# pyscf/pyscf

Measured on AMD Instinct MI355X. Metric: ms per SCF iter (DF J/K build), lower is better.
Workload: dtype f64

## Files before the change

pyscf_amd/csrc/xc_sparse.hip:

```cpp
#include <algorithm>
#include <type_traits>
#include <vector>
#include "common.h"
#include "mfma_e2.h"

using namespace pamd;

static int g_orb_dot_dma = 1;
static int g_orb_rho_128 = 1;
static int g_orb_rho_fused = 1;
static int g_vmat_probe = 0;
static int g_vmat_burst = 0;
static int g_vmat_even = 1;
static int g_vmat_flip = 0;
static int g_vmat_xcd = 1;

namespace {

struct SubTiles {
    const long *ao_off;
    const long *aow_off;
    const long *idx_off;
    const int *ld;
    const int *idx;
};


__device__ __forceinline__ int xcd_contiguous(int b, int n, int enabled)
{
    if (!enabled || n < 16) return b;
    const int q = n >> 3, r = n & 7, x = b & 7, slot = b >> 3;
    return x < r ? x * (q + 1) + slot : r * (q + 1) + (x - r) * q + slot;
}

template <int MT>
__global__ __launch_bounds__(256, 2) void sub_orb_dot_kernel(const double *__restrict__ ao_c, SubTiles tl, int G, int nchunk,
                                                             const double *__restrict__ orb, int ldo, int nocc_pad,
                                                             double *__restrict__ cmo, long comp_stride, long ldc)
{
    const int t = blockIdx.z / nchunk, chunk = blockIdx.z - t * nchunk;
    const int ld = tl.ld[t];
    const double *src = ao_c + tl.ao_off[t] + (long)blockIdx.y * G * ld;
    double *out = cmo + (long)blockIdx.y * comp_stride + (long)t * G;
    e2_symm_body<MT, true, true>(src, ld, ld, orb, ldo, out, nocc_pad, ldc, G, nullptr, nullptr, tl.idx + tl.idx_off[t],
                                 blockIdx.x * NT, chunk * (MT * 16));
}

__global__ __launch_bounds__(256, 2) void sub_orb_dot2_kernel(const double *__restrict__ ao_c, SubTiles tl, int G, int nchunk,
                                                              const double *__restrict__ orb, int ldo, int nocc_pad,
                                                              double *__restrict__ cmo, long comp_stride, long ldc)
{
    __shared__ double sa0[KB * LDN + KB * 32];
    __shared__ double sa1[KB * LDN + KB * 32];
    __shared__ double sq0[KB * LDN];
    __shared__ double sq1[KB * LDN];
    constexpr int RB = KB * LDN;
    const int tid = threadIdx.x, lane = tid & 63;
    const int wave = __builtin_amdgcn_readfirstlane(tid >> 6);
    const int t = blockIdx.z / nchunk, chunk = blockIdx.z - t * nchunk;
    const int ld = tl.ld[t];
    const int n0 = blockIdx.x * NT, m0 = chunk * 160;
    const int *idx = tl.idx + tl.idx_off[t];
    const __amdgpu_buffer_rsrc_t r_b = __builtin_amdgcn_make_buffer_rsrc(
        (void *)(ao_c + tl.ao_off[t] + ((long)blockIdx.y * G + n0) * ld), 0, 0xffffffff, 0x00020000);
    const __amdgpu_buffer_rsrc_t r_orb = __builtin_amdgcn_make_buffer_rsrc((void *)(orb + m0), 0, 0xffffffff, 0x00020000);
    const int ldo8 = ldo * 8;
    const int voff = lane * 16;
    const int rrow = lane >> 4;
    const int voff_remcol = (128 + ((((lane & 15) * 2) - 16 * (rrow & 1)) & 31)) * 8;
    const int wr = wave >> 1, wc = wave & 1;
    const int fk = lane >> 4, fn = lane & 15;
    const int offa = fk * LDN + wr * 64 + fn;
    const int offr = RB + fk * 32 + ((wr * 16 + fn + 16 * (fk & 1)) & 31);
    const int pl = fn & 7, bodd = (fn >> 3) & 1;
    const int offb_tr = (wc * 8 + (fn >> 3)) * 128 + (((pl ^ bodd) * 8) + ((fk >> 1) ^ (pl & 1))) * 2 + (fk & 1);
    int atr[4];
#pragma unroll
    for (int g = 0; g < 4; g++) atr[g] = offb_tr + (((2 * g) ^ (pl & 6))) * 2;
    int voff_tr[4];
#pragma unroll
    for (int j = 0; j < 4; j++) {
        const int blk = wave * 4 + j;
        const int pl_s = (lane >> 3) ^ (blk & 1);
        const int kp = (lane & 7) ^ pl_s;
        voff_tr[j] = ((blk * 8 + pl_s) * ld + 2 * kp) * 8;
    }

    double4_t acc[5][4];
#pragma unroll
    for (int a = 0; a < 5; a++)
#pragma unroll
        for (int b = 0; b < 4; b++) acc[a][b] = double4_t{0, 0, 0, 0};

    auto stage_row = [&](int k0, double *da, double *db, int j) {
        const int k = wave * 4 + j;
        const int row = idx[k0 + k];
        __builtin_amdgcn_raw_ptr_buffer_load_lds(r_orb, (__attribute__((address_space(3))) void *)(da + k * LDN), 16, voff, row * ldo8, 0, 0);
        __builtin_amdgcn_raw_ptr_buffer_load_lds(r_b, (__attribute__((address_space(3))) void *)(db + k * 128), 16, voff_tr[j], k0 * 8, 0, 0);
        if (j == 0) {
            const int rowl = idx[k0 + wave * 4 + rrow];
            __builtin_amdgcn_raw_ptr_buffer_load_lds(r_orb, (__attribute__((address_space(3))) void *)(da + RB + wave * 128), 16,
                                                     rowl * ldo8 + voff_remcol, 0, 0, 0);
        }
    };
    auto step = [&](const double *ca, const double *cb, double *na, double *nb, int k0) {
        asm volatile("s_waitcnt vmcnt(0)" ::: "memory");
        __syncthreads();
        const int kn = (k0 + KB < ld) ? k0 + KB : k0;
#pragma unroll
        for (int kk = 0; kk < KB; kk += 4) {
            double af[5], bf[4];
#pragma unroll
            for (int a = 0; a < 4; a++) af[a] = ca[offa + kk * LDN + a * 16];
            af[4] = ca[offr + kk * 32];
#pragma unroll
            for (int b = 0; b < 4; b++) bf[b] = cb[atr[kk >> 2] + b * 256];
            stage_row(kn, na, nb, kk >> 2);
#pragma unroll
            for (int a = 0; a < 5; a++)
#pragma unroll
                for (int b = 0; b < 4; b++) acc[a][b] = mfma_f64_16x16x4(af[a], bf[b], acc[a][b]);
        }
    };
#pragma unroll
    for (int j = 0; j < 4; j++) stage_row(0, sa0, sq0, j);
    for (int k0 = 0; k0 < ld; k0 += 2 * KB) {
        step(sa0, sq0, sa1, sq1, k0);
        if (k0 + KB < ld) step(sa1, sq1, sa0, sq0, k0 + KB);
    }
    double *out = cmo + (long)blockIdx.y * comp_stride + (long)t * G;
#pragma unroll
    for (int a = 0; a < 5; a++)
#pragma unroll
        for (int b = 0; b < 4; b++) {
            const int n = n0 + wc * 64 + b * 16 + fn;
            if (n >= G) continue;
#pragma unroll
            for (int r = 0; r < 4; r++) {
                const int i = m0 + (a < 4 ? wr * 64 + a * 16 : 128 + wr * 16) + fk + 4 * r;
                if (i < nocc_pad) out[(long)i * ldc + n] = acc[a][b][r];
            }
        }
}

template <bool REM>
__global__ __launch_bounds__(256, 2) void sub_orb_rho_kernel(const double *__restrict__ ao_c, SubTiles tl, int G, int nchunk,
                                                             const double *__restrict__ orb, int ldo, int nocc,
                                                             const double *__restrict__ sign, double *__restrict__ rho, long ldg)
{
    constexpr int NA = REM ? 5 : 4, CW = REM ? 160 : 128;
    __shared__ double sa0[KB * LDN + KB * 32];
    __shared__ double sa1[KB * LDN + KB * 32];
    __shared__ double sq0[KB * LDN];
    __shared__ double sq1[KB * LDN];
    constexpr int RB = KB * LDN;
    const int tid = threadIdx.x, lane = tid & 63;
    const int wave = __builtin_amdgcn_readfirstlane(tid >> 6);
    const int t = blockIdx.z / nchunk, chunk = blockIdx.z - t * nchunk;
    const int ld = tl.ld[t];
    const int g0 = blockIdx.x * 32, m0 = chunk * CW;
    const int *idx = tl.idx + tl.idx_off[t];
    const __amdgpu_buffer_rsrc_t r_b = __builtin_amdgcn_make_buffer_rsrc((void *)(ao_c + tl.ao_off[t] + (long)g0 * ld), 0, 0xffffffff,
                                                                        0x00020000);
    const __amdgpu_buffer_rsrc_t r_orb = __builtin_amdgcn_make_buffer_rsrc((void *)(orb + m0), 0, 0xffffffff, 0x00020000);
    const int ldo8 = ldo * 8;
    const int voff = lane * 16;
    const int rrow = lane >> 4;
    const int voff_remcol = (128 + ((((lane & 15) * 2) - 16 * (rrow & 1)) & 31)) * 8;
    const int wr = wave >> 1, wc = wave & 1;
    const int fk = lane >> 4, fn = lane & 15;
    const int offa = fk * LDN + wr * 64 + fn;
    const int offr = RB + fk * 32 + ((wr * 16 + fn + 16 * (fk & 1)) & 31);
    const int pl = fn & 7, bodd = (fn >> 3) & 1;
    const int offb_tr = (wc * 8 + (fn >> 3)) * 128 + (((pl ^ bodd) * 8) + ((fk >> 1) ^ (pl & 1))) * 2 + (fk & 1);
    int atr[4];
#pragma unroll
    for (int g = 0; g < 4; g++) atr[g] = offb_tr + (((2 * g) ^ (pl & 6))) * 2;
    int voff_tr[4];
#pragma unroll
    for (int j = 0; j < 4; j++) {
        const int blk = wave * 4 + j;
        const int pl_s = (lane >> 3) ^ (blk & 1);
        const int kp = (lane & 7) ^ pl_s;
        const int n = blk * 8 + pl_s;
        const int comp = (n >> 4) & 3, pt = ((n >> 6) << 4) | (n & 15);
        voff_tr[j] = (int)((((long)comp * G + pt) * ld + 2 * kp) * 8);
    }

    double4_t acc[NA][4];
#pragma unroll
    for (int a = 0; a < NA; a++)
#pragma unroll
        for (int b = 0; b < 4; b++) acc[a][b] = double4_t{0, 0, 0, 0};

    auto stage_row = [&](int k0, double *da, double *db, int j) {
        const int k = wave * 4 + j;
        const int row = idx[k0 + k];
        __builtin_amdgcn_raw_ptr_buffer_load_lds(r_orb, (__attribute__((address_space(3))) void *)(da + k * LDN), 16, voff, row * ldo8, 0, 0);
        __builtin_amdgcn_raw_ptr_buffer_load_lds(r_b, (__attribute__((address_space(3))) void *)(db + k * 128), 16, voff_tr[j], k0 * 8, 0, 0);
        if (REM && j == 0) {
            const int rowl = idx[k0 + wave * 4 + rrow];
            __builtin_amdgcn_raw_ptr_buffer_load_lds(r_orb, (__attribute__((address_space(3))) void *)(da + RB + wave * 128), 16,
                                                     rowl * ldo8 + voff_remcol, 0, 0, 0);
        }
    };
    auto step = [&](const double *ca, const double *cb, double *na, double *nb, int k0) {
        asm volatile("s_waitcnt vmcnt(0)" ::: "memory");
        __syncthreads();
        const int kn = (k0 + KB < ld) ? k0 + KB : k0;
#pragma unroll
        for (int kk = 0; kk < KB; kk += 4) {
            double af[NA], bf[4];
#pragma unroll
            for (int a = 0; a < 4; a++) af[a] = ca[offa + kk * LDN + a * 16];
            if (REM) af[NA - 1] = ca[offr + kk * 32];
#pragma unroll
            for (int b = 0; b < 4; b++) bf[b] = cb[atr[kk >> 2] + b * 256];
            stage_row(kn, na, nb, kk >> 2);
#pragma unroll
            for (int a = 0; a < NA; a++)
#pragma unroll
                for (int b = 0; b < 4; b++) acc[a][b] = mfma_f64_16x16x4(af[a], bf[b], acc[a][b]);
        }
    };
#pragma unroll
    for (int j = 0; j < 4; j++) stage_row(0, sa0, sq0, j);
    for (int k0 = 0; k0 < ld; k0 += 2 * KB) {
        step(sa0, sq0, sa1, sq1, k0);
        if (k0 + KB < ld) step(sa1, sq1, sa0, sq0, k0 + KB);
    }
    double p0 = 0, px = 0, py = 0, pz = 0;
#pragma unroll
    for (int a = 0; a < NA; a++)
#pragma unroll
        for (int r = 0; r < 4; r++) {
            const int i = m0 + (a < 4 ? wr * 64 + a * 16 : 128 + wr * 16) + fk + 4 * r;
            const double c0 = acc[a][0][r];
            const double w = (sign != nullptr && i < nocc) ? sign[i] * c0 : c0;
            p0 += w * c0;
            px += w * acc[a][1][r];
            py += w * acc[a][2][r];
            pz += w * acc[a][3][r];
        }
#pragma unroll
    for (int off = 16; off < 64; off <<= 1) {
        p0 += __shfl_xor(p0, off, 64);
        px += __shfl_xor(px, off, 64);
        py += __shfl_xor(py, off, 64);
        pz += __shfl_xor(pz, off, 64);
    }
    asm volatile("s_waitcnt vmcnt(0)" ::: "memory");
    __syncthreads();
    double *part = sa0;
    if (fk == 0) {
        part[(wave * 4 + 0) * 16 + fn] = p0;
        part[(wave * 4 + 1) * 16 + fn] = 2.0 * px;
        part[(wave * 4 + 2) * 16 + fn] = 2.0 * py;
        part[(wave * 4 + 3) * 16 + fn] = 2.0 * pz;
    }
    __syncthreads();
    if (tid < 128) {
        const int c = tid >> 5, pt = tid & 31, wcol = pt >> 4, f = pt & 15;
        const double v = part[((0 * 2 + wcol) * 4 + c) * 16 + f] + part[((1 * 2 + wcol) * 4 + c) * 16 + f];
        double *dst = rho + (long)c * ldg + (long)t * G + g0 + pt;
        if (nchunk == 1) *dst = v;
        else unsafeAtomicAdd(dst, v);
    }
}

__global__ __launch_bounds__(256) void sub_scale_kernel(const double *__restrict__ ao_c, SubTiles tl, int G, int ncomp,
                                                        const double *__restrict__ wv, long ldg, double *__restrict__ aow_c)
{
    const int t = blockIdx.z;
    const int ld = tl.ld[t];
    const int m = blockIdx.x * 256 + threadIdx.x;
    if (m >= ld) return;
    const long g = blockIdx.y;
    const double *a = ao_c + tl.ao_off[t] + g * ld + m;
    const long cs = (long)G * ld;
    const long gg = (long)t * G + g;
    double v = wv[gg] * a[0];
    if (ncomp == 4) v += wv[ldg + gg] * a[cs] + wv[2 * ldg + gg] * a[2 * cs] + wv[3 * ldg + gg] * a[3 * cs];
    aow_c[tl.aow_off[t] + g * ld + m] = v;
}

__global__ __launch_bounds__(256, 2) void sub_vmat_kernel(const double *__restrict__ ao_c, const double *__restrict__ aow_c,
                                                          SubTiles tl, const int *__restrict__ work, int G, int nao,
                                                          double *__restrict__ vmat, long ldv, int xcd)
{
    __shared__ double sb0[2 * KB * LDN];
    __shared__ double sb1[2 * KB * LDN];
    constexpr int PA = KB * LDN;
    const int tid = threadIdx.x, lane = tid & 63;
    const int wave = __builtin_amdgcn_readfirstlane(tid >> 6);
    const int item = xcd_contiguous(blockIdx.x, gridDim.x, xcd);
    const int t = work[3 * item], tm = work[3 * item + 1], tn = work[3 * item + 2];
    const int ld = tl.ld[t];
    const int p0 = tm * NT, q0 = tn * NT;
    const __amdgpu_buffer_rsrc_t r_a = __builtin_amdgcn_make_buffer_rsrc((void *)(ao_c + tl.ao_off[t] + p0), 0, 0xffffffff, 0x00020000);
    const __amdgpu_buffer_rsrc_t r_b = __builtin_amdgcn_make_buffer_rsrc((void *)(aow_c + tl.aow_off[t] + q0), 0, 0xffffffff, 0x00020000);
    const int voff = lane * 16, ld8 = ld * 8;
    const int wr = wave >> 1, wc = wave & 1;
    const int fk = lane >> 4, fn = lane & 15;
    const int offa = fk * LDN + wr * 64 + fn, offb = PA + fk * LDN + wc * 64 + fn;

    int na = (ld - (p0 + wr * 64) + 15) / 16, nb = (ld - (q0 + wc * 64) + 15) / 16;
    na = na < 0 ? 0 : (na > 4 ? 4 : na);
    nb = nb < 0 ? 0 : (nb > 4 ? 4 : nb);

    double4_t acc[4][4];
#pragma unroll
    for (int a = 0; a < 4; a++)
#pragma unroll
        for (int b = 0; b < 4; b++) acc[a][b] = double4_t{0, 0, 0, 0};

    auto stage_row = [&](int k0, double *dst, int j) {
        const int k = wave * 4 + j;
        __builtin_amdgcn_raw_ptr_buffer_load_lds(r_a, (__attribute__((address_space(3))) void *)(dst + k * LDN), 16, voff, (k0 + k) * ld8, 0, 0);
        __builtin_amdgcn_raw_ptr_buffer_load_lds(r_b, (__attribute__((address_space(3))) void *)(dst + PA + k * LDN), 16, voff, (k0 + k) * ld8, 0, 0);
    };
    auto kloop = [&](auto NAc, auto NBc) {
        constexpr int NA = decltype(NAc)::value, NB = decltype(NBc)::value;
        auto step = [&](const double *cur, double *nxt, int k0) {
            asm volatile("s_waitcnt vmcnt(0)" ::: "memory");
            __syncthreads();
            const int kn = (k0 + KB < G) ? k0 + KB : k0;
#pragma unroll
            for (int kk = 0; kk < KB; kk += 4) {
                double af[4], bf[4];
#pragma unroll
                for (int a = 0; a < NA; a++) af[a] = cur[offa + kk * LDN + a * 16];
#pragma unroll
                for (int b = 0; b < NB; b++) bf[b] = cur[offb + kk * LDN + b * 16];
                stage_row(kn, nxt, kk >> 2);
#pragma unroll
                for (int a = 0; a < NA; a++)
#pragma unroll
                    for (int b = 0; b < NB; b++) acc[a][b] = mfma_f64_16x16x4(af[a], bf[b], acc[a][b]);
            }
        };
        for (int k0 = 0; k0 < G; k0 += 2 * KB) {
            step(sb0, sb1, k0);
            if (k0 + KB < G) step(sb1, sb0, k0 + KB);
        }
    };
#pragma unroll
    for (int j = 0; j < 4; j++) stage_row(0, sb0, j);
    using I0 = std::integral_constant<int, 0>;
    using I1 = std::integral_constant<int, 1>;
    using I2 = std::integral_constant<int, 2>;
    using I3 = std::integral_constant<int, 3>;
    using I4 = std::integral_constant<int, 4>;
    auto pick_b = [&](auto NAc) {
        switch (nb) {
        case 1: kloop(NAc, I1{}); break;
        case 2: kloop(NAc, I2{}); break;
        case 3: kloop(NAc, I3{}); break;
        default: kloop(NAc, I4{}); break;
        }
    };
    if (na == 0 || nb == 0) {
        kloop(I0{}, I0{});
        asm volatile("s_waitcnt vmcnt(0)" ::: "memory");
        return;
    }
    switch (na) {
    case 1: pick_b(I1{}); break;
    case 2: pick_b(I2{}); break;
    case 3: pick_b(I3{}); break;
    default: pick_b(I4{}); break;
    }
    const int *idx = tl.idx + tl.idx_off[t];
#pragma unroll
    for (int b = 0; b < 4; b++) {
        const int col = q0 + wc * 64 + b * 16 + fn;
        if (col >= ld) continue;
        const int aj = idx[col];
        if (aj >= nao) continue;
#pragma unroll
        for (int a = 0; a < 4; a++)
#pragma unroll
            for (int r = 0; r < 4; r++) {
                const int rowi = p0 + wr * 64 + a * 16 + fk + 4 * r;
                if (rowi >= ld) continue;
                const int ai = idx[rowi];
                if (ai < nao) unsafeAtomicAdd(vmat + (long)ai * ldv + aj, acc[a][b][r]);
            }
    }
}

template <bool BURST, int PROBE>
__global__ __launch_bounds__(256, 2) void sub_vmat_sym_kernel(const double *__restrict__ ao_c, const double *__restrict__ aow_c,
                                                              SubTiles tl, const int *__restrict__ work, int G, int nao,
                                                              double *__restrict__ vmat, long ldv, int flip)
{
    __shared__ double sb0[2 * KB * LDN];
    __shared__ double sb1[2 * KB * LDN];
    constexpr int PA = KB * LDN;
    const int tid = threadIdx.x, lane = tid & 63;
    const int wave = __builtin_amdgcn_readfirstlane(tid >> 6);
    const int *w = work + 6 * (long)blockIdx.x;
    const int t = w[0], p0 = w[1], gp = w[2], q0 = w[3], gq = w[4], diag = w[5];
    if (gp == 0) return;
    const int ld = tl.ld[t];
    const int voff = lane * 16, ld8 = ld * 8;
    const int role = wave ^ ((flip == 1 ? (blockIdx.x >> 3) & 1 : flip == 2 ? (blockIdx.x >> 8) & 1 : 0) ? 3 : 0);
    const int wr = role >> 1, wc = role & 1;
    const int fk = lane >> 4, fn = lane & 15;
    const int ga0 = (gp + 1) >> 1, gb0 = (gq + 1) >> 1;
    const int na = wr == 0 ? ga0 : gp - ga0, nb = wc == 0 ? gb0 : gq - gb0;
    const int ra = wr * ga0 * 16, cb = wc * gb0 * 16;
    const int offa = fk * LDN + ra + fn, offb = PA + fk * LDN + cb + fn;
    const double *A = ao_c + tl.ao_off[t], *W = aow_c + tl.aow_off[t];
    const int nphase = diag ? 1 : 2;

    double4_t acc[4][4];
#pragma unroll
    for (int a = 0; a < 4; a++)
#pragma unroll
        for (int b = 0; b < 4; b++) acc[a][b] = double4_t{0, 0, 0, 0};

    auto kloop = [&](auto NAc, auto NBc) {
        constexpr int NA = decltype(NAc)::value, NB = decltype(NBc)::value;
        for (int ph = 0; ph < nphase; ph++) {
            const __amdgpu_buffer_rsrc_t r_a = __builtin_amdgcn_make_buffer_rsrc((void *)((ph ? W : A) + p0), 0, 0xffffffff, 0x00020000);
            const __amdgpu_buffer_rsrc_t r_b = __builtin_amdgcn_make_buffer_rsrc((void *)((ph ? A : W) + q0), 0, 0xffffffff, 0x00020000);
            auto stage_row = [&](int k0, double *dst, int j) {
                const int k = wave * 4 + j;
                __builtin_amdgcn_raw_ptr_buffer_load_lds(r_a, (__attribute__((address_space(3))) void *)(dst + k * LDN), 16, voff, (k0 + k) * ld8, 0, 0);
                __builtin_amdgcn_raw_ptr_buffer_load_lds(r_b, (__attribute__((address_space(3))) void *)(dst + PA + k * LDN), 16, voff, (k0 + k) * ld8, 0, 0);
            };
            auto step = [&](const double *cur, double *nxt, int k0) {
                asm volatile("s_waitcnt vmcnt(0)" ::: "memory");
                __syncthreads();
                const int kn = (k0 + KB < G) ? k0 + KB : k0;
#pragma unroll
                for (int kk = 0; kk < KB; kk += 4) {
                    double af[4], bf[4];
#pragma unroll
                    for (int a = 0; a < NA; a++) af[a] = cur[offa + kk * LDN + a * 16];
#pragma unroll
                    for (int b = 0; b < NB; b++) bf[b] = cur[offb + kk * LDN + b * 16];
                    if (PROBE == 2) {
                    } else if (BURST) {
                        if (kk == 0) {
#pragma unroll
                            for (int j = 0; j < 4; j++) stage_row(kn, nxt, j);
                        }
                    } else {
                        stage_row(kn, nxt, kk >> 2);
                    }
                    if (PROBE == 3) {
                        acc[0][0][0] += af[0] + bf[0];
                        continue;
                    }
#pragma unroll
                    for (int a = 0; a < NA; a++)
#pragma unroll
                        for (int b = 0; b < NB; b++) acc[a][b] = mfma_f64_16x16x4(af[a], bf[b], acc[a][b]);
                }
            };
            __syncthreads();
#pragma unroll
            for (int j = 0; j < 4; j++) stage_row(0, sb0, j);
            for (int k0 = 0; k0 < G; k0 += 2 * KB) {
                step(sb0, sb1, k0);
                if (k0 + KB < G) step(sb1, sb0, k0 + KB);
            }
            asm volatile("s_waitcnt vmcnt(0)" ::: "memory");
        }
    };
    using I0 = std::integral_constant<int, 0>;
    using I1 = std::integral_constant<int, 1>;
    using I2 = std::integral_constant<int, 2>;
    using I3 = std::integral_constant<int, 3>;
    using I4 = std::integral_constant<int, 4>;
    auto pick_b = [&](auto NAc) {
        switch (nb) {
        case 1: kloop(NAc, I1{}); break;
        case 2: kloop(NAc, I2{}); break;
        case 3: kloop(NAc, I3{}); break;
        default: kloop(NAc, I4{}); break;
        }
    };
    if (na <= 0 || nb <= 0) {
        kloop(I0{}, I0{});
        return;
    }
    switch (na) {
    case 1: pick_b(I1{}); break;
    case 2: pick_b(I2{}); break;
    case 3: pick_b(I3{}); break;
    default: pick_b(I4{}); break;
    }
    if (PROBE == 1) {
        double sum = 0;
#pragma unroll
        for (int a = 0; a < 4; a++)
#pragma unroll
            for (int b = 0; b < 4; b++) sum += acc[a][b][0] + acc[a][b][1] + acc[a][b][2] + acc[a][b][3];
        if (sum == 1.2345e300) vmat[0] = 1;
        return;
    }
    const int *idx = tl.idx + tl.idx_off[t];
#pragma unroll
    for (int b = 0; b < 4; b++) {
        if (b >= nb) continue;
        const int col = q0 + cb + b * 16 + fn;
        if (col >= ld) continue;
        const int aj = idx[col];
        if (aj >= nao) continue;
#pragma unroll
        for (int a = 0; a < 4; a++) {
            if (a >= na) continue;
#pragma unroll
            for (int r = 0; r < 4; r++) {
                const int rowi = p0 + ra + a * 16 + fk + 4 * r;
                if (rowi >= ld) continue;
                const int ai = idx[rowi];
                if (ai >= nao) continue;
                if (!diag) unsafeAtomicAdd(vmat + (long)ai * ldv + aj, acc[a][b][r]);
                else if (rowi > col) unsafeAtomicAdd(vmat + (long)ai * ldv + aj, acc[a][b][r]);
                else if (rowi < col) unsafeAtomicAdd(vmat + (long)aj * ldv + ai, acc[a][b][r]);
                else unsafeAtomicAdd(vmat + (long)ai * ldv + aj, 2.0 * acc[a][b][r]);
            }
        }
    }
}

__global__ void mirror_tril_kernel(const double *__restrict__ part, int m, int ldc, double *__restrict__ out)
{
    const int j = blockIdx.x * blockDim.x + threadIdx.x;
    const int i = blockIdx.y;
    if (j >= m) return;
    out[(long)i * m + j] = i >= j ? part[(long)i * ldc + j] : part[(long)j * ldc + i];
}

__global__ __launch_bounds__(256) void sub_gather_kernel(const double *__restrict__ dense, long dense_rows, int ldao,
                                                         int ncomp, long row0, long nrows_valid, SubTiles tl, int G,
                                                         int nao, double *__restrict__ ao_c)
{
    const int t = blockIdx.z;
    const int ld = tl.ld[t];
    const int m = blockIdx.x * 256 + threadIdx.x;
    if (m >= ld) return;
    const long g = blockIdx.y;
    const long row = row0 + (long)t * G + g;
    const int mu = tl.idx[tl.idx_off[t] + m];
    const bool ok = row < nrows_valid && mu < nao;
    for (int c = 0; c < ncomp; c++)
        ao_c[tl.ao_off[t] + ((long)c * G + g) * ld + m] = ok ? dense[((long)c * dense_rows + row) * ldao + mu] : 0.0;
}

}

extern "C" {

int PAMD_set_tuning_xc(const char *key, int value)
{
    if (strcmp(key, "orbdotdma") == 0) { g_orb_dot_dma = value; return 0; }
    if (strcmp(key, "orbrho") == 0) { g_orb_rho_fused = value; return 0; }
    if (strcmp(key, "orbrho128") == 0) { g_orb_rho_128 = value; return 0; }
    if (strcmp(key, "vmatxcd") == 0) { g_vmat_xcd = value; return 0; }
    if (strcmp(key, "vmatflip") == 0) { g_vmat_flip = value; return 0; }
    if (strcmp(key, "vmateven") == 0) { g_vmat_even = value; return 0; }
    if (strcmp(key, "vmatburst") == 0) { g_vmat_burst = value; return 0; }
    if (strcmp(key, "vmatprobe") == 0) { g_vmat_probe = value; return 0; }
    return pamd::set_error(-3, "unknown tuning key", __FILE__, __LINE__);
}


int PAMD_sub_orb_dot(const double *d_ao_c, const long *d_ao_off, const long *d_idx_off, const int *d_ld, const int *d_idx,
                     int ntile, int G, int ncomp, const double *d_orb, int ldo, int nocc_pad, double *d_cmo,
                     long comp_stride, long ldc, void *stream)
{
    PAMD_REQUIRE(nocc_pad % 16 == 0 && nocc_pad <= ldo, "nocc_pad must be a multiple of 16 and <= ldo");
    PAMD_REQUIRE(G % NT == 0, "tile size must be a multiple of 128");
    if (ntile == 0 || nocc_pad == 0) return 0;
    const int mt_total = nocc_pad / 16;
    const int nchunk = ceil_div(mt_total, 10);
    const int mt = ceil_div(mt_total, nchunk);
    PAMD_REQUIRE(ldo >= nchunk * mt * 16, "orbital leading dimension too small for tile padding");
    PAMD_REQUIRE((long)ntile * nchunk < 65536, "too many tiles per call");
    SubTiles tl{d_ao_off, nullptr, d_idx_off, d_ld, d_idx};
    dim3 grid(G / NT, ncomp, ntile * nchunk);
    hipStream_t st = (hipStream_t)stream;
    if (g_orb_dot_dma && mt >= 8 && ldo >= nchunk * 160 && ldo % 2 == 0 && (uintptr_t)d_orb % 16 == 0 &&
        (uintptr_t)d_ao_c % 16 == 0) {
        sub_orb_dot2_kernel<<<grid, 256, 0, st>>>(d_ao_c, tl, G, nchunk, d_orb, ldo, nocc_pad, d_cmo, comp_stride, ldc);
        PAMD_CHECK_LAUNCH();
        return 0;
    }
#define LAUNCH_S(MT) sub_orb_dot_kernel<MT><<<grid, 256, 0, st>>>(d_ao_c, tl, G, nchunk, d_orb, ldo, nocc_pad, d_cmo, comp_stride, ldc)
    switch (mt) {
    case 1: LAUNCH_S(1); break;
    case 2: LAUNCH_S(2); break;
    case 3: LAUNCH_S(3); break;
    case 4: LAUNCH_S(4); break;
    case 5: LAUNCH_S(5); break;
    case 6: LAUNCH_S(6); break;
    case 7: LAUNCH_S(7); break;
    case 8: LAUNCH_S(8); break;
    case 9: LAUNCH_S(9); break;
    default: LAUNCH_S(10); break;
    }
#undef LAUNCH_S
    PAMD_CHECK_LAUNCH();
    return 0;
}

int PAMD_sub_orb_rho(const double *d_ao_c, const long *d_ao_off, const long *d_idx_off, const int *d_ld, const int *d_idx,
                     int ntile, int G, const double *d_orb, int ldo, int nocc, int nocc_pad, const double *d_sign, double *d_rho,
                     long ldg, void *stream)
{
    PAMD_REQUIRE(nocc_pad % 16 == 0 && nocc_pad <= ldo, "nocc_pad must be a multiple of 16 and <= ldo");
    PAMD_REQUIRE(G % NT == 0, "tile size must be a multiple of 128");
    if (ntile == 0 || nocc_pad == 0) return 0;
    const int mt_total = nocc_pad / 16;
    int nchunk = ceil_div(mt_total, 10);
    const int mt = ceil_div(mt_total, nchunk);
    const int n128 = ceil_div(mt_total, 8);
    const bool narrow = g_orb_rho_128 && n128 * 8 < nchunk * 10 && ldo >= n128 * 128 + 32;
    if (narrow) nchunk = n128;
    if (!(g_orb_rho_fused && g_orb_dot_dma && mt >= 8 && ldo >= nchunk * (narrow ? 128 : 160) && ldo % 2 == 0 && (uintptr_t)d_orb % 16 == 0 &&
          (uintptr_t)d_ao_c % 16 == 0 && (long)ntile * nchunk < 65536))
        return 1;
    SubTiles tl{d_ao_off, nullptr, d_idx_off, d_ld, d_idx};
    dim3 grid(G / 32, 1, ntile * nchunk);
    if (narrow) sub_orb_rho_kernel<false><<<grid, 256, 0, (hipStream_t)stream>>>(d_ao_c, tl, G, nchunk, d_orb, ldo, nocc, d_sign, d_rho, ldg);
    else sub_orb_rho_kernel<true><<<grid, 256, 0, (hipStream_t)stream>>>(d_ao_c, tl, G, nchunk, d_orb, ldo, nocc, d_sign, d_rho, ldg);
    PAMD_CHECK_LAUNCH();
    return 0;
}

int PAMD_sub_scale_ao(const double *d_ao_c, const long *d_ao_off, const long *d_aow_off, const int *d_ld, int ntile, int G,
                      int ncomp, int ld_max, const double *d_wv, long ldg, double *d_aow_c, void *stream)
{
    if (ntile == 0) return 0;
    PAMD_REQUIRE(ntile < 65536 && G < 65536, "grid limits");
    SubTiles tl{d_ao_off, d_aow_off, nullptr, d_ld, nullptr};
    dim3 grid(ceil_div(ld_max, 256), G, ntile);
    sub_scale_kernel<<<grid, 256, 0, (hipStream_t)stream>>>(d_ao_c, tl, G, ncomp, d_wv, ldg, d_aow_c);
    PAMD_CHECK_LAUNCH();
    return 0;
}

int PAMD_sub_vmat(const double *d_ao_c, const long *d_ao_off, const double *d_aow_c, const long *d_aow_off,
                  const long *d_idx_off, const int *d_ld, const int *d_idx, const int *d_work, int nwork, int G, int nao,
                  double *d_vmat, long ldv, void *stream)
{
    PAMD_REQUIRE(G % (2 * KB) == 0 || G % KB == 0, "tile size must be a multiple of 16");
    PAMD_REQUIRE(((uintptr_t)d_ao_c | (uintptr_t)d_aow_c) % 16 == 0, "16-byte aligned operands");
    if (nwork == 0) return 0;
    SubTiles tl{d_ao_off, d_aow_off, d_idx_off, d_ld, d_idx};
    sub_vmat_kernel<<<nwork, 256, 0, (hipStream_t)stream>>>(d_ao_c, d_aow_c, tl, d_work, G, nao, d_vmat, ldv, g_vmat_flip);
    PAMD_CHECK_LAUNCH();
    return 0;
}

int PAMD_sub_vmat_sym(const double *d_ao_c, const long *d_ao_off, const double *d_aow_c, const long *d_aow_off,
                      const long *d_idx_off, const int *d_ld, const int *d_idx, const int *d_work, int nwork, int G, int nao,
                      double *d_vmat, long ldv, void *stream)
{
    PAMD_REQUIRE(G % KB == 0, "tile size must be a multiple of 16");
    PAMD_REQUIRE(((uintptr_t)d_ao_c | (uintptr_t)d_aow_c) % 16 == 0, "16-byte aligned operands");
    if (nwork == 0) return 0;
    SubTiles tl{d_ao_off, d_aow_off, d_idx_off, d_ld, d_idx};
    #define LAUNCH_VS(B, P) sub_vmat_sym_kernel<B, P><<<nwork, 256, 0, (hipStream_t)stream>>>(d_ao_c, d_aow_c, tl, d_work, G, nao, d_vmat, ldv, g_vmat_flip)
    if (g_vmat_probe == 1) LAUNCH_VS(false, 1);
    else if (g_vmat_probe == 2) LAUNCH_VS(false, 2);
    else if (g_vmat_probe == 3) LAUNCH_VS(false, 3);
    else if (g_vmat_burst) LAUNCH_VS(true, 0);
    else LAUNCH_VS(false, 0);
#undef LAUNCH_VS
    PAMD_CHECK_LAUNCH();
    return 0;
}

long PAMD_sub_vmat_work(const int *ld, int ntile, int *work)
{
    std::vector<int> order(ntile);
    for (int i = 0; i < ntile; i++) order[i] = i;
    std::stable_sort(order.begin(), order.end(), [&](int a, int b) { return ld[a] > ld[b]; });
    const int nq = g_vmat_xcd ? 8 : 1;
    std::vector<std::vector<int>> queue(nq);
    std::vector<double> load(nq, 0.0);
    for (int t : order) {
        const int g = ld[t] / 16, np = (g + 7) / 8;
        if (np == 0) continue;
        std::vector<int> first(np + 1, 0);
        if (g_vmat_even) {
            const int h = (g + 1) / 2, base = h / np, rem = h % np;
            for (int i = 0; i < np; i++) first[i + 1] = first[i] + 2 * (base + (i < rem ? 1 : 0)) - (i == 0 && (g & 1) ? 1 : 0);
        } else {
            const int base = g / np, rem = g % np;
            for (int i = 0; i < np; i++) first[i + 1] = first[i] + base + (i < rem ? 1 : 0);
        }
        int qi = 0;
        for (int k = 1; k < nq; k++) if (load[k] < load[qi]) qi = k;
        for (int i = 0; i < np; i++)
            for (int j = 0; j <= i; j++) {
                const int gp = first[i + 1] - first[i], gq = first[j + 1] - first[j];
                const int w[6] = {t, first[i] * 16, gp, first[j] * 16, gq, i == j};
                queue[qi].insert(queue[qi].end(), w, w + 6);
                load[qi] += ((gp + 1) / 2) * ((gq + 1) / 2) * (i == j ? 1 : 2);
            }
    }
    size_t depth = 0;
    for (auto &q : queue) depth = std::max(depth, q.size() / 6);
    const long n = (long)depth * nq;
    if (work) {
        for (size_t d = 0; d < depth; d++)
            for (int k = 0; k < nq; k++) {
                int *w = work + 6 * (d * nq + k);
                if (d * 6 < queue[k].size()) memcpy(w, &queue[k][d * 6], 6 * sizeof(int));
                else { w[0] = 0; w[1] = 0; w[2] = 0; w[3] = 0; w[4] = 0; w[5] = 0; }
            }
    }
    return n;
}

int PAMD_mirror_tril(const double *d_part, int m, int ldc, double *d_out, void *stream)
{
    dim3 grid(ceil_div(m, 256), m);
    mirror_tril_kernel<<<grid, 256, 0, (hipStream_t)stream>>>(d_part, m, ldc, d_out);
    PAMD_CHECK_LAUNCH();
    return 0;
}

int PAMD_sub_gather_ao(const double *d_dense, long dense_rows, int ldao, int ncomp, long row0, long nrows_valid,
                       const long *d_ao_off, const long *d_idx_off, const int *d_ld, const int *d_idx, int ntile, int G,
                       int ld_max, int nao, double *d_ao_c, void *stream)
{
    if (ntile == 0) return 0;
    PAMD_REQUIRE(ntile < 65536 && G < 65536, "grid limits");
    SubTiles tl{d_ao_off, nullptr, d_idx_off, d_ld, d_idx};
    dim3 grid(ceil_div(ld_max, 256), G, ntile);
    sub_gather_kernel<<<grid, 256, 0, (hipStream_t)stream>>>(d_dense, dense_rows, ldao, ncomp, row0, nrows_valid, tl, G, nao,
                                                           d_ao_c);
    PAMD_CHECK_LAUNCH();
    return 0;
}

}
```

Measured before the change: 112.3.

## Add two-phase orbital-rho kernel computing gradient via weighted second GEMM

```diff
diff --git a/pyscf_amd/csrc/xc_sparse.hip b/pyscf_amd/csrc/xc_sparse.hip
--- a/pyscf_amd/csrc/xc_sparse.hip
+++ b/pyscf_amd/csrc/xc_sparse.hip
@@ -8,7 +8,7 @@
 
 static int g_orb_dot_dma = 1;
 static int g_orb_rho_128 = 1;
-static int g_orb_rho_fused = 1;
+static int g_orb_rho_fused = 2;
 static int g_vmat_probe = 0;
 static int g_vmat_burst = 0;
 static int g_vmat_even = 1;
@@ -268,6 +268,213 @@
     }
 }
 
+template <bool REM>
+__global__ __launch_bounds__(256, 2) void sub_orb_rho2_kernel(const double *__restrict__ ao_c, SubTiles tl, int G, int nchunk,
+                                                              const double *__restrict__ orb, int ldo, int nocc,
+                                                              const double *__restrict__ sign, double *__restrict__ rho, long ldg)
+{
+    constexpr int NA = REM ? 5 : 4, CW = REM ? 160 : 128;
+    constexpr int LD2 = NT + 4;
+    constexpr int SA = KB * LDN + KB * 32, SQ = KB * 96;
+    constexpr int RB = KB * LDN, RB2 = KB * LD2;
+    __shared__ double sa0[SA], sa1[SA];
+    __shared__ double sq0[SQ], sq1[SQ];
+    const int tid = threadIdx.x, lane = tid & 63;
+    const int wave = __builtin_amdgcn_readfirstlane(tid >> 6);
+    const int t = blockIdx.z / nchunk, chunk = blockIdx.z - t * nchunk;
+    const int ld = tl.ld[t];
+    const int g0 = blockIdx.x * 32, m0 = chunk * CW;
+    const int *idx = tl.idx + tl.idx_off[t];
+    const int ldo8 = ldo * 8;
+    const int voff = lane * 16;
+    const int rrow = lane >> 4;
+    const int voff_remcol = (128 + ((((lane & 15) * 2) - 16 * (rrow & 1)) & 31)) * 8;
+    const int voff_remcol2 = (128 + ((((lane & 15) * 2) - 4 * (wave * 4 + rrow)) & 31)) * 8;
+    const int wr = wave >> 1, wc = wave & 1;
+    const int fk = lane >> 4, fn = lane & 15;
+    const int offa = fk * LDN + wr * 64 + fn;
+    const int offr = RB + fk * 32 + ((wr * 16 + fn + 16 * (fk & 1)) & 31);
+    const int offa2 = fn * LD2 + wr * 64 + fk;
+    const int offr2 = RB2 + fn * 32;
+    const int colr2 = wr * 16 + fk + 4 * fn;
+    const int pl = fn & 7, bodd = (fn >> 3) & 1;
+    const int offb_in = (((pl ^ bodd) * 8) + ((fk >> 1) ^ (pl & 1))) * 2 + (fk & 1);
+    int atr1[4], atr[4];
+#pragma unroll
+    for (int g = 0; g < 4; g++) {
+        atr1[g] = (wc * 2 + (fn >> 3)) * 128 + offb_in + (((2 * g) ^ (pl & 6))) * 2;
+        atr[g] = (wc * 6 + (fn >> 3)) * 128 + offb_in + (((2 * g) ^ (pl & 6))) * 2;
+    }
+    int voff_tr[3];
+#pragma unroll
+    for (int j = 0; j < 3; j++) {
+        const int blk = wave * 3 + j;
+        const int pl_s = (lane >> 3) ^ (blk & 1);
+        const int kp = (lane & 7) ^ pl_s;
+        const int n = blk * 8 + pl_s;
+        const int wcol = n / 48, comp = 1 + ((n - wcol * 48) >> 4), pt = (wcol << 4) | (n & 15);
+        voff_tr[j] = (int)((((long)comp * G + pt) * ld + 2 * kp) * 8);
+    }
+    int voff_b1;
+    {
+        const int pl_s = (lane >> 3) ^ (wave & 1);
+        const int kp = (lane & 7) ^ pl_s;
+        voff_b1 = ((wave * 8 + pl_s) * ld + 2 * kp) * 8;
+    }
+
+    typedef int int4_t __attribute__((ext_vector_type(4)));
+    auto make_rsrc = [](const void *ptr) {
+        const unsigned long u = (unsigned long)ptr;
+        return int4_t{(int)(unsigned)u, (int)(unsigned)(u >> 32), -1, 0x00020000};
+    };
+    const int4_t q_b = make_rsrc(ao_c + tl.ao_off[t] + (long)g0 * ld), q_orb = make_rsrc(orb + m0);
+    auto dma = [&](const int4_t &rsrc, const double *dst, int voffset, int soffset) {
+        const unsigned lds = (unsigned)(unsigned long)dst;
+        asm volatile("s_mov_b32 m0, %0\n\ts_nop 0\n\tbuffer_load_dwordx4 %1, %2, %3 offen lds"
+                     :: "s"(lds), "v"(voffset), "s"(rsrc), "s"(soffset) : "memory");
+    };
+    const __attribute__((address_space(4))) int *idxc = (const __attribute__((address_space(4))) int *)idx;
+    int row_a[4];
+    auto load_rows = [&](int k0) {
+#pragma unroll
+        for (int j = 0; j < 4; j++) row_a[j] = idxc[k0 + wave * 4 + j];
+    };
+    auto rem_row = [&]() { return rrow == 0 ? row_a[0] : rrow == 1 ? row_a[1] : rrow == 2 ? row_a[2] : row_a[3]; };
+    auto stage1 = [&](int k0, double *da, double *db, int j) {
+        dma(q_orb, da + (wave * 4 + j) * LDN, voff, row_a[j] * ldo8);
+        if (j == 1)
+            dma(q_b, db + wave * 128, voff_b1, k0 * 8);
+        if (REM && j == 0)
+            dma(q_orb, da + RB + wave * 128, rem_row() * ldo8 + voff_remcol, 0);
+    };
+    auto stage2 = [&](int k0, double *da, double *db, int j) {
+        dma(q_orb, da + (wave * 4 + j) * LD2, voff, row_a[j] * ldo8);
+        if (j < 3)
+            dma(q_b, db + (wave * 3 + j) * 128, voff_tr[j < 3 ? j : 0], k0 * 8);
+        if (REM && j == 0)
+            dma(q_orb, da + RB2 + wave * 128, rem_row() * ldo8 + voff_remcol2, 0);
+    };
+
+    double4_t acc[NA];
+#pragma unroll
+    for (int a = 0; a < NA; a++) acc[a] = double4_t{0, 0, 0, 0};
+    const int nk = ld / KB, ns = 2 * nk;
+    auto buf_a = [&](auto I) -> double * { return I.value == 0 ? sa0 : sa1; };
+    auto buf_q = [&](auto I) -> double * { return I.value == 0 ? sq0 : sq1; };
+    auto stage = [&](int s, auto I, int j) {
+        if (s >= ns) return;
+        if (s < nk) stage1(s * KB, buf_a(I), buf_q(I), j);
+        else stage2((s - nk) * KB, buf_a(I), buf_q(I), j);
+    };
+    auto next_rows = [&](int s) {
+        if (s < ns) load_rows((s < nk ? s : s - nk) * KB);
+    };
+    double p0 = 0, px = 0, py = 0, pz = 0;
+    auto mult1 = [&](int s, auto I, auto N) {
+        const double *ca = buf_a(I), *cb = buf_q(I);
+#pragma unroll
+        for (int kk = 0; kk < KB; kk += 4) {
+            double af[NA];
+#pragma unroll
+            for (int a = 0; a < 4; a++) af[a] = ca[offa + kk * LDN + a * 16];
+            if (REM) af[NA - 1] = ca[offr + kk * 32];
+            const double bf = cb[atr1[kk >> 2]];
+            stage(s + 1, N, kk >> 2);
+#pragma unroll
+            for (int a = 0; a < NA; a++) acc[a] = mfma_f64_16x16x4(af[a], bf, acc[a]);
+        }
+    };
+    auto weights = [&]() {
+        double sg[NA][4];
+        if (sign != nullptr) {
+#pragma unroll
+            for (int a = 0; a < NA; a++)
+#pragma unroll
+                for (int r = 0; r < 4; r++) {
+                    const int i = m0 + (a < 4 ? wr * 64 + a * 16 : 128 + wr * 16) + fk + 4 * r;
+                    sg[a][r] = sign[i < nocc ? i : nocc - 1];
+                }
+        }
+#pragma unroll
+        for (int a = 0; a < NA; a++)
+#pragma unroll
+            for (int r = 0; r < 4; r++) {
+                const double c0 = acc[a][r];
+                const double w = sign != nullptr ? sg[a][r] * c0 : c0;
+                p0 += w * c0;
+                acc[a][r] = w;
+            }
+    };
+    auto mult2 = [&](int s, auto I, auto N) {
+        const double *ca = buf_a(I), *cb = buf_q(I);
+        double4_t t0 = double4_t{0, 0, 0, 0}, t1 = double4_t{0, 0, 0, 0};
+#pragma unroll
+        for (int a = 0; a < NA; a++) {
+            double af[4];
+#pragma unroll
+            for (int r = 0; r < 4; r++)
+                af[r] = a < 4 ? ca[offa2 + a * 16 + 4 * r] : ca[offr2 + ((colr2 + 4 * r) & 31)];
+            if (a < 4) stage(s + 1, N, a);
+#pragma unroll
+            for (int r = 0; r < 4; r++) {
+                if (r & 1) t1 = mfma_f64_16x16x4(af[r], acc[a][r], t1);
+                else t0 = mfma_f64_16x16x4(af[r], acc[a][r], t0);
+            }
+        }
+#pragma unroll
+        for (int r = 0; r < 4; r++) {
+            const double tt = t0[r] + t1[r];
+            px += tt * cb[atr[r]];
+            py += tt * cb[atr[r] + 256];
+            pz += tt * cb[atr[r] + 512];
+        }
+    };
+    auto step = [&](int s, auto I) {
+        std::integral_constant<int, 1 - I.value> N;
+        asm volatile("s_waitcnt vmcnt(0)" ::: "memory");
+        __syncthreads();
+        if (s < nk) mult1(s, I, N);
+        else {
+            if (s == nk) weights();
+            mult2(s, I, N);
+        }
+        next_rows(s + 2);
+    };
+    std::integral_constant<int, 0> I0;
+    std::integral_constant<int, 1> I1;
+    next_rows(0);
+#pragma unroll
+    for (int j = 0; j < 4; j++) stage(0, I0, j);
+    next_rows(1);
+    for (int s = 0; s < ns; s += 2) {
+        step(s, I0);
+        step(s + 1, I1);
+    }
+#pragma unroll
+    for (int off = 16; off < 64; off <<= 1) {
+        p0 += __shfl_xor(p0, off, 64);
+        px += __shfl_xor(px, off, 64);
+        py += __shfl_xor(py, off, 64);
+        pz += __shfl_xor(pz, off, 64);
+    }
+    __syncthreads();
+    double *part = sa0;
+    if (fk == 0) {
+        part[(wave * 4 + 0) * 16 + fn] = p0;
+        part[(wave * 4 + 1) * 16 + fn] = 2.0 * px;
+        part[(wave * 4 + 2) * 16 + fn] = 2.0 * py;
+        part[(wave * 4 + 3) * 16 + fn] = 2.0 * pz;
+    }
+    __syncthreads();
+    if (tid < 128) {
+        const int c = tid >> 5, pt = tid & 31, wcol = pt >> 4, f = pt & 15;
+        const double v = part[((0 * 2 + wcol) * 4 + c) * 16 + f] + part[((1 * 2 + wcol) * 4 + c) * 16 + f];
+        double *dst = rho + (long)c * ldg + (long)t * G + g0 + pt;
+        if (nchunk == 1) *dst = v;
+        else unsafeAtomicAdd(dst, v);
+    }
+}
+
 __global__ __launch_bounds__(256) void sub_scale_kernel(const double *__restrict__ ao_c, SubTiles tl, int G, int ncomp,
                                                         const double *__restrict__ wv, long ldg, double *__restrict__ aow_c)
 {
@@ -627,8 +834,15 @@
         return 1;
     SubTiles tl{d_ao_off, nullptr, d_idx_off, d_ld, d_idx};
     dim3 grid(G / 32, 1, ntile * nchunk);
-    if (narrow) sub_orb_rho_kernel<false><<<grid, 256, 0, (hipStream_t)stream>>>(d_ao_c, tl, G, nchunk, d_orb, ldo, nocc, d_sign, d_rho, ldg);
-    else sub_orb_rho_kernel<true><<<grid, 256, 0, (hipStream_t)stream>>>(d_ao_c, tl, G, nchunk, d_orb, ldo, nocc, d_sign, d_rho, ldg);
+#define LAUNCH_R(KERNEL, REM) KERNEL<REM><<<grid, 256, 0, (hipStream_t)stream>>>(d_ao_c, tl, G, nchunk, d_orb, ldo, nocc, d_sign, d_rho, ldg)
+    if (g_orb_rho_fused >= 2) {
+        if (narrow) LAUNCH_R(sub_orb_rho2_kernel, false);
+        else LAUNCH_R(sub_orb_rho2_kernel, true);
+    } else {
+        if (narrow) LAUNCH_R(sub_orb_rho_kernel, false);
+        else LAUNCH_R(sub_orb_rho_kernel, true);
+    }
+#undef LAUNCH_R
     PAMD_CHECK_LAUNCH();
     return 0;
 }
```

Measured after the change: 112.6. About the same (+0.2%).
